# tsurumeso/vocal-remover

Hardware: AMD Instinct MI355X
Metric: spectrogram-frames/sec (inference, CascadedNet n_fft=2048) (higher is better)
Workload: dtype f32; 1 GPU; configs[1]: 30 s stereo 44.1 kHz synthetic song, STFT -> 11 crops of 256 frames in one device batch -> predict_mask -> stitch -> mask apply -> iSTFT x2; n_fft=2048, hop=1024, cropsize=256, parallelism=replicas x1 (songs shard, no collective), input_residency=inputs resident in HBM when the timed region starts

## Files before the change

vocal-remover_amd/csrc/kernels.h:

```cpp
#pragma once
#include "vr_common.h"

namespace vr {

struct HeadDst {
    float* p;
    long long dN, dC, dH;
    int w_lo, w_hi;
    int pad_rows;
    float* const* items;
    const int* item_pitch;
};
void launch_head_sigmoid(const Tensor& x, const float* w , const HeadDst& d, hipStream_t st);
void launch_head_complex(const Tensor& x, const float* w , const HeadDst& d, hipStream_t st);
int launch_squeeze_conv(const Tensor& x, const float* w , float* out, float* part, bool dry, hipStream_t st,
                        const float* epi = nullptr);

void launch_avgpool_h(const Tensor& x, float* out, hipStream_t st);

struct BNFoldDesc { const float *w, *b, *rm, *rv; float* affine; int C; int bcast; };
void launch_bn_fold_eval(const BNFoldDesc* d_descs, int ndesc, int maxC, float eps, hipStream_t st);
struct BNFinalizeArgs {
    const float* part; int nparts; int pstride;
    double count;
// ... 119 lines not shown
void launch_head_loss(const Tensor& x, const float* w, const float* X, const float* Y, int bins, float gscale,
                      float* dlogit, float* mask_out, float* loss_part, float* loss_out, float loss_scale, hipStream_t st);
void launch_head_bwd(const float* dmask, const float* mask, int N, int H, int W, int bins, float* dlogit, hipStream_t st);
void launch_head_loss_complex(const Tensor& x, const float* w, const float* X, const float* Y, int bins, float gscale,
                              float* dlogit, float* mask_out, float* loss_part, float* loss_out, float loss_scale, hipStream_t st);
void launch_head_bwd_complex(const Tensor& x, const float* w, const float* dmask, int bins, float* dlogit, hipStream_t st);
struct MagL1 {};
void launch_head_mag_l1(const Tensor& x, const float* w, const float* X, const float* Y, int bins, float* mask_out, float* loss_part,
                        float* loss_out, float loss_scale, hipStream_t st);
struct FlipDesc { const float* w; float* wt; int Cin, Cout, KK, CinPad, CoutPad; };
void launch_flip_transpose(const FlipDesc* d_descs, int n, hipStream_t st);
void launch_adam(float* p, const float* g, float* m, float* v, long long n, double lr, double b1, double b2, double eps,
                 long long step, double gscale, hipStream_t st);
void launch_channel_sum(const float* d, int N, int C, int W, float* out, int accumulate, hipStream_t st);
void launch_f32_to_bf16(const float* x, unsigned short* y, long long n, hipStream_t st);
void launch_bf16_to_f32(const unsigned short* x, float* y, long long n, hipStream_t st);

void launch_mul_crop(const float* x, float* m, bool cplx, long long rows, int T, int Wm, int off, hipStream_t st);
int l1_crop_blocks();
enum L1CropForm { L1_CROP_REAL = 0, L1_CROP_COMPLEX = 1, L1_CROP_MAG = 2 };
void launch_l1_crop(L1CropForm form, const float* pred, const float* y, long long rows, int T, int Wm, int off, float* part, float* loss,
                    hipStream_t st);

struct FFTPlan { int n_fft; int log2n; float2* twiddle; float* window; };
void launch_stft(const FFTPlan& pl, const float* wave, long long L, int hop, int T, float2* spec, hipStream_t st);
void launch_istft(const FFTPlan& pl, const float2* spec, int hop, int T, float* frames, float* wave, hipStream_t st);
bool istft_masked_available(const FFTPlan& pl, int hop);
void launch_istft_masked(const FFTPlan& pl, const float2* spec, int hop, int T, const float* mask_a, int Wa, const float* mask_b,
                         int Wb, int shift, const float* wgt, int which, float* wave, hipStream_t st);
struct PcmIn { const uint8_t* bytes; int channels; int fmt; };
void launch_stft_pcm(const FFTPlan& pl, const PcmIn& in, long long L, int T, float2* spec, hipStream_t st);
void launch_istft_masked_pcm16(const FFTPlan& pl, const float2* spec, int hop, int T, bool cplx, const float* mask_a, int Wa,
                               const float* mask_b, int Wb, int shift, const float* wgt, int which, int16_t* out, hipStream_t st);
void launch_mag_pad(const float2* spec, int bins, int T, float* mag_pad, int Wpad, int pad_l,
                    unsigned* stats, hipStream_t st);
void launch_coef_affine(unsigned* stats, int rows, int mode, float* aff, hipStream_t st);
void launch_coef_complex(unsigned* stats, int rows, int mode, float2* inv, hipStream_t st);
void launch_pack_complex(const float2* spec, int N, int bins, int T, float* dst, int Wdst, int pad_l, const float2* scale,
                         hipStream_t st);
void launch_apply_mask(const float2* spec, int bins, int T, const float* mask_a, int Wa,
                       const float* mask_b, int Wb, int shift, const float* wgt, float2* y, float2* v, hipStream_t st);
void launch_frame_min(int bins, int T, const float* mask_a, int Wa, const float* mask_b, int Wb, int shift, float* fmin,
                      hipStream_t st);
void launch_apply_mask_complex(const float2* spec, int bins, int T, const float2* mask_a, int Wa, const float2* mask_b, int Wb,
                               int shift, const float* wgt, float2* y, float2* v, hipStream_t st);
void launch_istft_masked_complex(const FFTPlan& pl, const float2* spec, int hop, int T, const float2* mask_a, int Wa,
                                 const float2* mask_b, int Wb, int shift, const float* wgt, int which, float* wave, hipStream_t st);
// ... 155 lines not shown
```

vocal-remover_amd/csrc/model.h:

```cpp
#pragma once
#include <chrono>
#include <deque>
#include <functional>
#include <map>
#include <memory>
#include <string>
#include <vector>

#include "kernels.h"
#include "weight_forms.h"

namespace vr {

struct Arena {
    char* base = nullptr;
    size_t cap = 0, off = 0, peak = 0;
    bool dry = false;
    void* alloc(size_t bytes) {
        const size_t a = (off + 255) & ~size_t(255);
        off = a + bytes;
        if (off > peak) peak = off;
        if (dry) return reinterpret_cast<void*>(uintptr_t(256));
        if (off > cap) throw Error(-4, "workspace arena overflow (planning bug)");
        return base + a;
// ... 250 lines not shown
    int net_w_lo = 0, net_w_hi = 0;
    void set_option(const std::string& name, int value);
    void reset_adam_state();
    void profile_end(double* conv_ms, double* conv_flops, double* conv_bytes, int* launches);

    hipStream_t stream = nullptr;
    hipStream_t side_stream = nullptr;
    hipEvent_t ev_fork = nullptr, ev_join = nullptr;
    bool band_fork_active = false;
    bool gs_clear_pending = false;
    bool wgrad_on_side = false;
    struct Lane { hipStream_t main = nullptr, side = nullptr; hipEvent_t fork = nullptr, join = nullptr, start = nullptr, done = nullptr; Arena ws; };
    std::vector<Lane> lanes;
    void swap_lane(int i);

private:
    float* p_arena = nullptr; size_t p_floats = 0;
    float* b_arena = nullptr; size_t b_floats = 0;
    Arena ws;
    Arena io;
    void ensure_ws(size_t bytes);
    int plan_B = -1, plan_T = -1; bool plan_training = false; size_t plan_peak = 0;
    void ensure_io(size_t bytes);

    std::deque<BN> bns;
    std::vector<BN*> bn_list;
    struct PendingConv { ConvArgs a; ConvShape shp; double flops, bytes; bool stats; BNFinalizeArgs fin; BN* bn; };
    std::vector<PendingConv>* conv_sink = nullptr;
    int x3d_mode = 2;
    int conv_w_lo = 0, conv_w_hi = 0;
    int x3s_mode = x3s_default();
    static int x3s_default() { const char* e = getenv("VR_CONV_X3S"); return (e && atoi(e) == 0) ? 0 : 1; }
    FormStore form_store;
    void hold_form(FormId f, const std::vector<Conv*>& convs, Wino6Want w6, FormStore& s);
    void fill_form(FormId f, const std::vector<Conv*>& convs, Wino6Want w6, FormStore& s, bool single);
    FormSelect form_select() const { return FormSelect{mfma_mode, training, train_wino, x3d_mode, x3s_mode, dry}; }
    std::vector<WgReduceDesc> wred_host, wred_sent;
    WgReduceDesc* wred_dev = nullptr;
    size_t wred_cap = 0;
    void flush_wgrad_sums();
    static long long x3_batch_max_elems(const std::vector<X3WDesc>& descs);
    static int x3_batch_max_cout_pad(const std::vector<X3WDesc>& descs);
    static long long wino_batch_max_elems(const std::vector<WinoWDesc>& descs, bool split6);
    static long long s2w_batch_max_elems(const std::vector<S2WDesc>& descs);
    void refresh_forms(bool with_dgrad);
    BNFoldDesc* d_fold = nullptr;
// ... 131 lines not shown
```

vocal-remover_amd/csrc/model.hip:

```cpp
#include "pcm.h"
#include "model.h"

#include <algorithm>
#include <chrono>
#include <cmath>
#include <cstdlib>
#include <cstring>

namespace vr {

static inline int round_up(int v, int m) { return (v + m - 1) / m * m; }

Param* Model::add_param(const std::string& key, std::vector<int64_t> shape, ParamKind kind, bool trainable) {
    params.emplace_back();
    Param* p = &params.back();
    p->key = key;
    p->shape = std::move(shape);
    p->kind = kind;
    p->trainable = trainable;
    p->numel = 1;
    for (auto d : p->shape) p->numel *= (size_t)d;
    p->dev_numel = p->numel;
    if (kind == PK_CONV) {
        p->Cout = (int)p->shape[0];
// ... 123 lines not shown
    build_basenet(nets_[2], "stg2_low_band_net.0", nout / 4 + nin, nout, nin_lstm / 2, nout_lstm);
    build_cba(tail2, "stg2_low_band_net.1", nout, nout / 2, 1, 1, 0, 0, 1, 1, 0.f);
    build_basenet(nets_[3], "stg2_high_band_net", nout / 4 + nin, nout / 2, nin_lstm / 2, nout_lstm / 2);
    build_basenet(nets_[4], "stg3_full_band_net", 3 * nout / 4 + nin, nout, nin_lstm, nout_lstm);
    out_w = add_param("out.weight", {nin, nout, 1, 1}, PK_PLAIN, true);
    aux_out_w = add_param("aux_out.weight", {nin, 3 * nout / 4, 1, 1}, PK_PLAIN, true);
    finalize_layout();

    plan.n_fft = n_fft;
    plan.log2n = 0;
    while ((1 << plan.log2n) < n_fft) ++plan.log2n;
    std::vector<float2> tw(n_fft / 2);
    std::vector<float> win(n_fft);
    const double PI = 3.14159265358979323846;
    for (int k = 0; k < n_fft / 2; ++k) {
        const double a = -2.0 * PI * k / n_fft;
        tw[k] = make_float2((float)std::cos(a), (float)std::sin(a));
    }
    for (int i = 0; i < n_fft; ++i) win[i] = (float)(0.5 - 0.5 * std::cos(2.0 * PI * i / n_fft));
    VR_HIP(hipMalloc(&plan.twiddle, tw.size() * sizeof(float2)));
    VR_HIP(hipMalloc(&plan.window, win.size() * sizeof(float)));
    VR_HIP(hipMemcpy(plan.twiddle, tw.data(), tw.size() * sizeof(float2), hipMemcpyHostToDevice));
    VR_HIP(hipMemcpy(plan.window, win.data(), win.size() * sizeof(float), hipMemcpyHostToDevice));
}

void Model::finalize_layout() {
    size_t poff = 0, boff = 0;
    auto bump = [](size_t& o, size_t n) { size_t a = (o + 63) & ~size_t(63); o = a + n; return a; };
    for (auto& p : params) {
        if (p.kind == PK_NBT || p.alias_of) continue;
        if (p.trainable) p.off = bump(poff, p.dev_numel);
        else p.off = bump(boff, p.dev_numel);
    }
    std::vector<size_t> aff_off(bn_list.size()), sm_off(bn_list.size()), si_off(bn_list.size());
    for (size_t i = 0; i < bn_list.size(); ++i) {
        BN* b = bn_list[i];
        const int rows = b->bcast ? b->bcast : b->C;
        aff_off[i] = bump(boff, (size_t)rows * 2);
        sm_off[i] = bump(boff, (size_t)b->C);
        si_off[i] = bump(boff, (size_t)b->C);
    }
    size_t aspp_off[5];
    for (int i = 0; i < 5; ++i) aspp_off[i] = bump(boff, (size_t)4 * 8 * nets_[i].c * 2);
    p_floats = poff + 64; b_floats = boff + 64;
    VR_HIP(hipMalloc(&p_arena, p_floats * sizeof(float)));
    VR_HIP(hipMalloc(&b_arena, b_floats * sizeof(float)));
// ... 20 lines not shown
    for (BN* b : bn_list) {
        std::vector<float> ones(b->C, 1.f);
        VR_HIP(hipMemcpy(b->w->dev, ones.data(), b->C * sizeof(float), hipMemcpyHostToDevice));
        VR_HIP(hipMemcpy(b->rv->dev, ones.data(), b->C * sizeof(float), hipMemcpyHostToDevice));
    }
    std::vector<BNFoldDesc> descs;
    for (BN* b : bn_list) descs.push_back(BNFoldDesc{b->w->dev, b->b->dev, b->rm->dev, b->rv->dev, b->affine, b->C, b->bcast});
    VR_HIP(hipMalloc(&d_fold, descs.size() * sizeof(BNFoldDesc)));
    VR_HIP(hipMemcpy(d_fold, descs.data(), descs.size() * sizeof(BNFoldDesc), hipMemcpyHostToDevice));
    affine_dirty = true;
}

Model::~Model() {
    if (launch_prof && !prof_owned_by_this_thread(launch_prof)) prof_abandon(launch_prof);
    else { if (g_launch_prof == launch_prof) g_launch_prof = nullptr; prof_destroy(launch_prof); }
    int prev_dev = -1;
    if (hipGetDevice(&prev_dev) != hipSuccess) prev_dev = -1;
    hipSetDevice(device);
    struct Back { int d; ~Back() { if (d >= 0) hipSetDevice(d); } } back{prev_dev};
    try { comm_destroy(); } catch (...) {}
    hipFree(wire_buf);
    if (stream) hipStreamSynchronize(stream);
    hipFree(p_arena); hipFree(b_arena); hipFree(d_fold);
    hipFree(ws.base); hipFree(io.base); hipFree(gs.base); form_store.release(); hipFree(aug_buf); hipFree(wred_dev);
    for (BaseNetL& B : nets_) hipFree(B.lstm.bias_sum);
    hipFree(g_arena); hipFree(m_arena); hipFree(v_arena); hipFree(dropout_buf);
    hipFree(plan.twiddle); hipFree(plan.window);
    for (Lane& l : lanes) {
        hipStreamSynchronize(l.main); hipStreamSynchronize(l.side);
        hipStreamDestroy(l.main); hipStreamDestroy(l.side);
        hipEventDestroy(l.fork); hipEventDestroy(l.join); hipEventDestroy(l.start); hipEventDestroy(l.done);
        hipFree(l.ws.base);
    }
    if (side_stream) { hipStreamSynchronize(side_stream); hipStreamDestroy(side_stream); hipEventDestroy(ev_fork); hipEventDestroy(ev_join); }
    if (stream) hipStreamDestroy(stream);
}

void Model::set_param(const std::string& key, const void* host, const int64_t* shape, int ndim) {
    auto it = by_key.find(key);
    VR_CHECK(it != by_key.end(), -2, "unknown parameter key: " + key);
    Param& p = *it->second;
    VR_CHECK((size_t)ndim == p.shape.size(), -2, "shape rank mismatch for " + key);
    for (int i = 0; i < ndim; ++i) VR_CHECK(shape[i] == p.shape[i], -2, "shape mismatch for " + key);
    DeviceGuard dev_guard(device);
    VR_HIP(hipStreamSynchronize(stream));
    if (p.kind == PK_NBT) { p.nbt = *static_cast<const int64_t*>(host); return; }
// ... 81 lines not shown

void Model::set_option(const std::string& name, int value) {
    plan_peak = 0;
    if (name == "train_winograd") train_wino = value != 0;
    else if (name == "serial_exec") serial = value != 0;
    else if (name == "params_dirty") affine_dirty = true;
    else if (name == "mfma_bf16") { mfma_mode = value != 0 ? 1 : default_mfma_mode; affine_dirty = true; }
    else if (name == "mfma_mode") {
        if (value < -1 || value > 3) throw Error(-2, "mfma_mode: 0, 1, 2, 3 or -1 (default)");
        mfma_mode = value < 0 ? default_mfma_mode : value; affine_dirty = true;
    }
    else if (name == "conv_x3d") {
        if (value < -1 || value > 2) throw Error(-2, "conv_x3d: 0, 1, 2 or -1 (default)");
        x3d_mode = value < 0 ? 2 : value;
    }
    else if (name == "conv_x3s") {
        if (value < -1 || value > 1) throw Error(-2, "conv_x3s: 0, 1 or -1 (default)");
        x3s_mode = value < 0 ? x3s_default() : value;
    }
    else if (name == "crop_window") crop_window = value != 0;
    else if (name == "fuse_tail") fuse_tail = value != 0;
    else if (name == "lstm_gemm") lstm_gemm = value != 0;
    else if (name == "aspp_pool_fused") aspp_pool_fused = value != 0;
    else if (name == "complex_train") {
        if (!is_complex) throw Error(-2, "complex_train: this handle predicts a magnitude mask; the option belongs to complex-mask handles (VR_CREATE_COMPLEX)");
        complex_train = value != 0;
        if (!complex_train && loss_kind != 0) set_loss(0, 0.01);
        graph_valid = false;
    }
    else if (name == "adam_reset") reset_adam_state();
    else if (name == "hip_graph" || name == "conv_x3p" || name == "wgrad_x3h" || name == "conv_x3b") {
        static std::string told;
        if (told.find("|" + name + "|") == std::string::npos) {
            told += "|" + name + "|";
            fprintf(stderr, "libvr_mi355: option '%s' was retired with its kernel (tools/experiments/README.md); ignored\n", name.c_str());
        }
    }
    else throw Error(-2, "unknown option: " + name);
}

void Model::hold_form(FormId f, const std::vector<Conv*>& convs, Wino6Want w6, FormStore& s) {
    if (s.arena[f]) return;
    auto room = [&](const Conv* L) {
        const FormSpec sp = form_spec(f, *L, mfma_mode, w6);
        return sp.held ? (sp.bytes + 255) & ~size_t(255) : size_t(0);
    };
// ... 89 lines not shown
    ws.base = nullptr; ws.cap = 0;
    const size_t want = bytes + (bytes >> 4) + (1 << 20);
    VR_HIP(hipMalloc(reinterpret_cast<void**>(&ws.base), want));
    ws.cap = want;
}

void Model::swap_lane(int i) {
    Lane& l = lanes[i];
    std::swap(stream, l.main);
    std::swap(side_stream, l.side);
    std::swap(ev_fork, l.fork);
    std::swap(ev_join, l.join);
    std::swap(ws, l.ws);
}

void Model::ensure_io(size_t bytes) {
    if (bytes <= io.cap) return;
    VR_HIP(hipStreamSynchronize(stream));
    if (io.base) VR_HIP(hipFree(io.base));
    io.base = nullptr; io.cap = 0;
    const size_t want = bytes + (bytes >> 4) + (1 << 20);
    VR_HIP(hipMalloc(reinterpret_cast<void**>(&io.base), want));
    io.cap = want;
}

double Model::conv_alg_bytes(const Conv& L, const ConvArgs& a, int N, bool batch_as_h) const {
    return 4.0 * ((double)a.N * L.Cin * a.Hin * a.Win + (double)N * L.Cout * (batch_as_h ? 1 : a.Hout) * a.Wout +
                  (double)L.Cin * L.KS * L.KS * L.Cout);
}

void Model::record_begin(int kind, double flops) {
    if (!profiling || dry) return;
    (void)kind;
    prof_note(flops, 0.0, true, "conv");
}
void Model::record_note(double bytes, const char* tag) {
    if (!profiling || dry || !g_launch_prof) return;
    prof_note_update(bytes, tag);
}
void Model::record_end() {
    if (!profiling || dry) return;
    prof_note_clear();
}

void Model::profile_begin() {
    VR_CHECK(!launch_prof || prof_owned_by_this_thread(launch_prof), -3, "vr_profile_begin: a profile opened by another thread is still open");
// ... 1132 lines not shown
    const int most = solo ? std::max(sg[0].patches[0], sg[0].patches[1]) : crops_n;
    const int bs = (batchsize <= 0) ? most : std::min(batchsize, most);
    const bool tiled = many_tiled_available(plan, hop);

    DeviceGuard dev_guard(device);
    std::vector<SongSeg> tab((size_t)n_songs);
    std::vector<float*> stage_in((size_t)n_songs), stage_y((size_t)n_songs), stage_v((size_t)n_songs);
    SongSeg* tab_d = nullptr; int2* crops_d = nullptr;
    std::vector<PcmIn> pin(pcm ? (size_t)n_songs : 0);
    PcmIn* pin_d = nullptr;
    std::vector<WaveEval> evt(eval ? (size_t)n_songs : 0);
    std::vector<float*> stage_inst(eval ? (size_t)n_songs : 0);
    WaveEval* evt_d = nullptr;
    std::vector<PseudoSeg> pst(pseudo ? (size_t)n_songs : 0);
    std::vector<float*> stage_pinst(pseudo ? (size_t)n_songs : 0);
    PseudoSeg* pst_d = nullptr;
    double pcm_bytes = 0.0;
    auto in_bytes = [&](int s) {
        return pcm ? (size_t)L[s] * pcm_channels[s] * pcm_sample_bytes(pcm_fmt[s]) : (waves ? (size_t)2 * L[s] : sg[s].spec_f) * sizeof(float);
    };
    unsigned long long* part = nullptr;
    float *aff = nullptr, *mask = nullptr, *gather = nullptr, *fmin_d = nullptr, *wgt_d = nullptr, *frames = nullptr;
    const size_t crop_f = (size_t)nin * max_bin * cropsize;
    auto carve = [&](Arena& A) {
        tab_d = static_cast<SongSeg*>(A.alloc(sizeof(SongSeg) * n_songs));
        crops_d = static_cast<int2*>(A.alloc(sizeof(int2) * crops_n));
        if (pcm) pin_d = static_cast<PcmIn*>(A.alloc(sizeof(PcmIn) * n_songs));
        if (eval) evt_d = static_cast<WaveEval*>(A.alloc(sizeof(WaveEval) * n_songs));
        if (pseudo) pst_d = static_cast<PseudoSeg*>(A.alloc(sizeof(PseudoSeg) * n_songs));
        part = static_cast<unsigned long long*>(A.alloc((size_t)n_songs * 2 * bins * 16));
        aff = A.allocf((size_t)n_songs * 4);
        mask = A.allocf((size_t)E * 2 * bins * W);
        gather = A.allocf((size_t)bs * crop_f + 4096);
        if (post) { fmin_d = A.allocf((size_t)sum_T); wgt_d = A.allocf((size_t)sum_T); }
        if (waves && !tiled) frames = A.allocf((size_t)2 * max_T * n_fft);
        for (int s = 0; s < n_songs; ++s) {
            const Song& g = sg[s];
            SongSeg& t = tab[s];
            t = SongSeg{};
            t.T = g.T;
            t.mcol_a = g.crop0[0] * roi;
            t.mcol_b = tta ? g.crop0[1] * roi + roi / 2 : 0;
            stage_in[s] = in_on_dev ? nullptr : A.allocf(in_bytes(s) / 4 + (pcm ? 1 : 0));
            const float* src = in_on_dev ? in[s] : stage_in[s];
            if (pseudo) {
                stage_pinst[s] = in_on_dev ? nullptr : A.allocf(in_bytes(s) / 4);
                const float* isrc = in_on_dev ? pseudo->inst[s] : stage_pinst[s];
                PseudoSeg& q = pst[s];
                q = PseudoSeg{};
// ... 37 lines not shown
                t.spec = reinterpret_cast<float2*>(const_cast<float*>(src));
                stage_y[s] = out_on_dev ? y[s] : A.allocf(g.spec_f);
                stage_v[s] = out_on_dev ? v[s] : A.allocf(g.spec_f);
                t.y = reinterpret_cast<float2*>(stage_y[s]); t.v = reinterpret_cast<float2*>(stage_v[s]);
            }
        }
    };
    Arena dry;
    dry.dry = true;
    carve(dry);
    ensure_io(dry.peak + 65536);
    io.reset();
    carve(io);
    std::vector<int2> crops((size_t)crops_n);
    int frame0 = 0;
    for (int s = 0; s < n_songs; ++s) {
        tab[s].frame0 = frame0;
        if (post) tab[s].fmin = fmin_d + frame0;
        frame0 += sg[s].T;
        for (int ps = 0; ps < (tta ? 2 : 1); ++ps)
            for (int i = 0; i < sg[s].patches[ps]; ++i)
                crops[(size_t)sg[s].crop0[ps] + i] = make_int2(s, i * roi - sg[s].pad_l - (ps ? roi / 2 : 0));
    }
    VR_HIP(hipMemcpyAsync(tab_d, tab.data(), sizeof(SongSeg) * n_songs, hipMemcpyHostToDevice, stream));
    VR_HIP(hipMemcpyAsync(crops_d, crops.data(), sizeof(int2) * crops_n, hipMemcpyHostToDevice, stream));
    if (pcm) {
        VR_HIP(hipMemcpyAsync(pin_d, pin.data(), sizeof(PcmIn) * n_songs, hipMemcpyHostToDevice, stream));
        for (int s = 0; s < n_songs; ++s) pcm_bytes += (double)in_bytes(s);
    }
    if (!in_on_dev)
        for (int s = 0; s < n_songs; ++s)
            VR_HIP(hipMemcpyAsync(stage_in[s], in[s], in_bytes(s), hipMemcpyHostToDevice, stream));
    if (eval) {
        VR_HIP(hipMemcpyAsync(evt_d, evt.data(), sizeof(WaveEval) * n_songs, hipMemcpyHostToDevice, stream));
        if (!in_on_dev)
            for (int s = 0; s < n_songs; ++s)
                VR_HIP(hipMemcpyAsync(stage_inst[s], eval->inst[s], in_bytes(s), hipMemcpyHostToDevice, stream));
    }
    if (pseudo) {
        VR_HIP(hipMemcpyAsync(pst_d, pst.data(), sizeof(PseudoSeg) * n_songs, hipMemcpyHostToDevice, stream));
        if (!in_on_dev)
            for (int s = 0; s < n_songs; ++s)
                VR_HIP(hipMemcpyAsync(stage_pinst[s], pseudo->inst[s], in_bytes(s), hipMemcpyHostToDevice, stream));
    }
    if (pseudo) {
        if (waves) launch_stft_pseudo_many(plan, tab_d, pst_d, n_songs, max_T, (double)sum_L, (double)sum_T, stream);
        else launch_pseudo_diff_many(tab_d, pst_d, n_songs, bins, (double)sum_T, stream);
    } else if (waves) {
// ... 559 lines not shown
```

vocal-remover_amd/csrc/stft.hip:

```cpp
#include "kernels.h"
#include "pcm.h"

#include <cfloat>
#include <cstdlib>
#include <cstring>
#include <type_traits>

namespace vr {

template <class SRC> constexpr bool kSongTable = std::is_same<SRC, const SongSeg>::value;
template <class SRC> constexpr bool kStream = std::is_same<SRC, const StreamSeg>::value;
template <class SRC> using StreamLocal = typename std::conditional<kStream<SRC>, StreamSeg, int>::type;
template <class SRC> constexpr bool kPair = std::is_same<SRC, const WavePair>::value;
template <class SRC> using PairLocal = typename std::conditional<kPair<SRC>, WavePair, int>::type;
template <class SRC> constexpr bool kTriple = std::is_same<SRC, const WaveTriple>::value;
template <class SRC> using TripleLocal = typename std::conditional<kTriple<SRC>, WaveTriple, int>::type;

__device__ __forceinline__ float stream_sample(const StreamSeg& sg, int ch, long long p) {
    if (p < 0 || p >= sg.L) return 0.f;
    return p < sg.blk_base ? sg.tail[(long long)ch * sg.tail_pitch + (p - sg.tail_base)] : sg.blk[(long long)ch * sg.blk_pitch + (p - sg.blk_base)];
}

__device__ __forceinline__ float2 cmul(float2 a, float2 b) {
    return make_float2(a.x * b.x - a.y * b.y, a.x * b.y + a.y * b.x);
}

__device__ __forceinline__ float2 sub_rounded(float2 a, float2 b) {
#pragma clang fp contract(off)
// ... 32 lines not shown
    for (int i = threadIdx.x; i < n; i += blockDim.x) {
        const long long p = start + i;
        const float v = (p >= 0 && p < L) ? wv[p] * pl.window[i] : 0.f;
        const int r = __brev((unsigned)i) >> (32 - pl.log2n);
        xs[r] = make_float2(v, 0.f);
    }
    fft_lds(xs, pl.twiddle, n, pl.log2n);
    const int bins = n / 2 + 1;
    for (int k = threadIdx.x; k < bins; k += blockDim.x)
        spec[((long long)ch * bins + k) * T + t] = xs[k];
}

void launch_stft(const FFTPlan& pl, const float* wave, long long L, int hop, int T, float2* spec, hipStream_t st);
static int tile_frames(const FFTPlan& pl, int extra_floats);
static bool tiled_signal_path(const FFTPlan& pl, int hop);
void launch_stft_tiled(const FFTPlan& pl, const float* wave, long long L, int T, float2* spec, hipStream_t st);

void launch_stft(const FFTPlan& pl, const float* wave, long long L, int hop, int T, float2* spec, hipStream_t st) {
    if (tiled_signal_path(pl, hop)) { launch_stft_tiled(pl, wave, L, T, spec, st); return; }
    VR_LAUNCH(stft_kernel, dim3(T, 2), dim3(256), pl.n_fft * sizeof(float2), st, pl, wave, L, hop, T, spec);
    VR_HIP(hipGetLastError());
}

__device__ __forceinline__ void fft_lds_sub(float2* x, const float2* __restrict__ tw, int n, int log2n, int twshift, int tid,
                                            int nt) {
    const int half_n = n >> 1;
    for (int s = 0; s < log2n; ++s) {
        const int half = 1 << s;
        __syncthreads();
        for (int b = tid; b < half_n; b += nt) {
            const int pos = b & (half - 1);
            const int i = ((b >> s) << (s + 1)) + pos;
            const int j = i + half;
            const float2 w = tw[(pos << (log2n - 1 - s)) << twshift];
            const float2 t = cmul(w, x[j]);
            const float2 u = x[i];
            x[i] = make_float2(u.x + t.x, u.y + t.y);
            x[j] = make_float2(u.x - t.x, u.y - t.y);
        }
    }
    __syncthreads();
}

constexpr int TG = 4;

template <class A> __device__ __forceinline__ A pcm_first(A a) { return a; }
template <class D, class... T> struct FirstOr { using type = D; };
template <class D, class A, class... T> struct FirstOr<D, A, T...> { using type = A; };

struct WaveF32In {
    const float* wv;
    __device__ __forceinline__ float at(long long p) const { return wv[p]; }
};
struct WavePcmIn {
    PcmIn in;
    int ch;
    __device__ __forceinline__ float at(long long p) const { return pcm_decode(in.bytes, in.fmt, in.channels, p, ch); }
};
struct WaveGradIn {
    const float* yw;
    const float* pw;
    const float* win;
// ... 20 lines not shown
        const float ws = fmaf(w0, w0, w2 * w2);
        const float a = fmaf(cy, yw[p], fmaf(cp, pw[p], cx * xw[p]));
        return ws > FLT_MIN ? a / ws : a;
    }
};
struct WaveF32Out {
    static constexpr bool kInterleaved = false;
    static __device__ __forceinline__ void put(float* w, long long pitch, int ch, long long p, int i, float v) { w[(long long)ch * pitch + p + i] = v; }
};
struct WavePcm16Out {
    static constexpr bool kInterleaved = true;
    static __device__ __forceinline__ void put(float* w, long long, int ch, long long p, int i, float v) {
        reinterpret_cast<int16_t*>(w)[(p + i) * 2 + ch] = pcm16_from_float(v);
    }
};

template <class SRC = const float, class... PCM>
__global__ __launch_bounds__(1024) void stft_tile_kernel(FFTPlan pl, SRC* __restrict__ wave, long long L, int T, int F,
                                                         float2* __restrict__ spec, PCM... pcm) {
    constexpr bool kGrad3 = std::is_same<typename FirstOr<void, PCM...>::type, WaveGrad3>::value;
    constexpr bool kGrad = std::is_same<typename FirstOr<void, PCM...>::type, WaveGrad>::value || kGrad3;
    constexpr bool kPseudo = std::is_same<typename FirstOr<void, PCM...>::type, const PseudoSeg*>::value;
    constexpr bool kPcm = sizeof...(PCM) == 1 && !kGrad && !kPseudo;
    static_assert(!kPseudo || kSongTable<SRC>, "the pair form is a song-table form");
    static_assert(sizeof...(PCM) <= 1 && !(sizeof...(PCM) == 1 && kStream<SRC>), "one PCM source at most, none for streams");
    extern __shared__ __attribute__((aligned(16))) float2 lds2[];
    const int n = pl.n_fft, M = n >> 1, bins = M + 1, hop = M, logM = pl.log2n - 1;
    const int g = threadIdx.x >> 8, tid = threadIdx.x & 255;
    float2* zs = lds2 + (size_t)g * M;
    float2* tile = lds2 + (size_t)TG * M;
    int t0 = blockIdx.x * F;
    const int ch = blockIdx.y;
    typename std::conditional<kPcm, WavePcmIn, typename std::conditional<kGrad3, WaveGrad3In,
                              typename std::conditional<kGrad, WaveGradIn, WaveF32In>::type>::type>::type in;
    typename std::conditional<kGrad3, WaveGrad3, typename std::conditional<kGrad, WaveGrad, int>::type>::type gd{};
    StreamLocal<SRC> ss{};
    typename std::conditional<kPseudo, PseudoSeg, int>::type ps{};
    const float* mix_wv = nullptr;
    if constexpr (kStream<SRC>) {
        ss = wave[blockIdx.z];
        if (blockIdx.x > 0 && t0 >= ss.T - ss.t_new) return;
        t0 += ss.t_new; T = ss.T;
        in.wv = nullptr;
    } else if constexpr (kSongTable<SRC>) {
        const SongSeg sg = wave[blockIdx.z];
        if (t0 >= sg.T) return;
// ... 11 lines not shown
                                             (double)gd.sums[4], (double)gd.sums[5]);
        in.xw = gd.x_wave + (long long)ch * L; in.yw = gd.y_wave + (long long)ch * L; in.pw = gd.p_wave + (long long)ch * L;
        in.win = pl.window; in.M = M;
        in.cy = (float)((double)gd.sdr_scale * c.cy); in.cp = (float)((double)gd.sdr_scale * c.cp); in.cx = (float)((double)gd.sdr_scale * c.cx);
    } else if constexpr (kGrad) {
        gd = pcm_first(pcm...);
        const double a = (double)gd.sums[0], p = sqrt((double)gd.sums[1]), q = sqrt((double)gd.sums[2]), D = p * q + 1e-8;
        in.yw = gd.y_wave + (long long)ch * L; in.pw = gd.p_wave + (long long)ch * L; in.win = pl.window; in.M = M;
        in.alpha = (float)(-(double)gd.sdr_scale / D);
        in.beta = q > 0.0 ? (float)((double)gd.sdr_scale * a * p / (q * D * D)) : 0.f;
    } else {
        if constexpr (kPcm) in.in = pcm_first(pcm...);
        else in.wv = wave + (long long)ch * L;
    }
    if constexpr (kPcm) in.ch = ch < in.in.channels ? ch : in.in.channels - 1;
    const int nf = (T - t0) < F ? (T - t0) : F;
    int pass = 0;
second_pass:
    for (int f0 = 0; f0 < nf; f0 += TG) {
        const int f = f0 + g;
        const bool live = f < nf;
        if (live) {
            const long long start = (long long)(t0 + f) * hop - M;
            for (int m = tid; m < M; m += 256) {
                const long long p = start + 2 * m;
                float v0, v1;
                if constexpr (kStream<SRC>) {
                    v0 = stream_sample(ss, ch, p) * pl.window[2 * m];
                    v1 = stream_sample(ss, ch, p + 1) * pl.window[2 * m + 1];
                } else {
                    v0 = (p >= 0 && p < L) ? in.at(p) * pl.window[2 * m] : 0.f;
                    v1 = (p + 1 >= 0 && p + 1 < L) ? in.at(p + 1) * pl.window[2 * m + 1] : 0.f;
                }
                zs[__brev((unsigned)m) >> (32 - logM)] = make_float2(v0, v1);
            }
        }
        fft_lds_sub(zs, pl.twiddle, M, logM, 1, tid, 256);
        if (live) {
            for (int k = tid; k < bins; k += 256) {
                const float2 zk = zs[k & (M - 1)], zm = zs[(M - k) & (M - 1)];
                const float2 e = make_float2(0.5f * (zk.x + zm.x), 0.5f * (zk.y - zm.y));
                const float2 b = make_float2(0.5f * (zk.x - zm.x), 0.5f * (zk.y + zm.y));
                const float2 w = k < M ? pl.twiddle[k] : make_float2(-1.f, 0.f);
                const float2 wb = cmul(w, b);
                if constexpr (kPseudo) {
                    const float2 xv = make_float2(e.x + wb.y, e.y - wb.x);
                    tile[k * F + f] = pass == 1 ? sub_rounded(xv, tile[k * F + f]) : xv;
                } else {
                    tile[k * F + f] = make_float2(e.x + wb.y, e.y - wb.x);
                }
            }
        }
// ... 358 lines not shown
        }
        __syncthreads();
        if (threadIdx.x < 6) {
            float s = 0.f;
            for (int w = 0; w < 16; ++w) s += red[w * 6 + threadIdx.x];
            tr.part[((long long)blockIdx.y * gridDim.x + blockIdx.x) * 6 + threadIdx.x] = s;
        }
    }
    if constexpr (kStream<SRC>) {
        if (t0 + nf == ss.t_done) {
            float* cout = ss.carry_out + (long long)(which * 2 + ch) * M;
            for (int i = threadIdx.x; i < M; i += 1024) cout[i] = prev[i];
        }
    }
}

static int tile_frames(const FFTPlan& pl, int extra_floats) {
    const int M = pl.n_fft / 2, bins = M + 1;
    long long budget = 150 * 1024 - (long long)TG * M * 8 - (long long)extra_floats * 4;
    int F = (int)(budget / ((long long)bins * 8));
    return F > 17 ? 17 : F;
}

static bool tiled_signal_path(const FFTPlan& pl, int hop) {
    static const bool on = !getenv("VR_NO_TILED_STFT");
    return on && hop * 2 == pl.n_fft && pl.n_fft >= 128 && tile_frames(pl, pl.n_fft / 2) >= 3;
}

template <bool CPLX, class... OUT>
static void launch_istft_tile(const FFTPlan& pl, const float2* spec, int hop, int T, const float* mask_a, int Wa, const float* mask_b,
                              int Wb, int shift, const float* wgt, int which, float* wave, hipStream_t st) {
    const int M = pl.n_fft / 2, bins = M + 1;
    const long long out_len = (long long)hop * (T - 1);
    if (out_len <= 0) return;
    const int F = tile_frames(pl, M);
    const int S = F - 1;
    const size_t lds = (size_t)TG * M * 8 + (size_t)bins * F * 8 + (size_t)M * 4;
    static std::atomic<unsigned long long> attr_done{0};
    ensure_lds_attr(attr_done, reinterpret_cast<const void*>(istft_tile_kernel<CPLX, const float2, OUT...>), 160 * 1024);
    prof_note(0.0, 2.0 * ((double)bins * T * (8.0 + (CPLX ? 8.0 : 4.0) * (mask_b ? 2 : 1)) + (sizeof...(OUT) ? 2.0 : 4.0) * (double)out_len));
    VR_LAUNCH((istft_tile_kernel<CPLX, const float2, OUT...>), dim3((unsigned)((T - 1 + S - 1) / S), 2), dim3(1024), lds, st, pl, spec, T, S, mask_a, Wa,
              mask_b, Wb, shift, wgt, which, wave, out_len);
    VR_HIP(hipGetLastError());
}

void launch_istft_masked(const FFTPlan& pl, const float2* spec, int hop, int T, const float* mask_a, int Wa, const float* mask_b,
                         int Wb, int shift, const float* wgt, int which, float* wave, hipStream_t st) {
    launch_istft_tile<false>(pl, spec, hop, T, mask_a, Wa, mask_b, Wb, shift, wgt, which, wave, st);
}

void launch_istft_masked_pcm16(const FFTPlan& pl, const float2* spec, int hop, int T, bool cplx, const float* mask_a, int Wa,
                               const float* mask_b, int Wb, int shift, const float* wgt, int which, int16_t* out, hipStream_t st) {
    float* w = reinterpret_cast<float*>(out);
    if (cplx) launch_istft_tile<true, WavePcm16Out>(pl, spec, hop, T, mask_a, Wa, mask_b, Wb, shift, wgt, which, w, st);
    else launch_istft_tile<false, WavePcm16Out>(pl, spec, hop, T, mask_a, Wa, mask_b, Wb, shift, wgt, which, w, st);
}

void launch_istft_masked_complex(const FFTPlan& pl, const float2* spec, int hop, int T, const float2* mask_a, int Wa,
                                 const float2* mask_b, int Wb, int shift, const float* wgt, int which, float* wave, hipStream_t st) {
    launch_istft_tile<true>(pl, spec, hop, T, reinterpret_cast<const float*>(mask_a), Wa, reinterpret_cast<const float*>(mask_b), Wb,
// ... 121 lines not shown
    const long long p = (long long)blockIdx.x * blockDim.x + threadIdx.x;
    const int ch = blockIdx.y;
    if (p >= out_len) return;
    const int n = pl.n_fft;
    const long long q = p + n / 2;
    long long t_hi = q / hop;
    if (t_hi > T - 1) t_hi = T - 1;
    long long t_lo = (q - n + hop) / hop;
    if (q - n + 1 <= 0) t_lo = 0;
    if (t_lo < 0) t_lo = 0;
    float acc = 0.f, wss = 0.f;
    for (long long t = t_lo; t <= t_hi; ++t) {
        const int i = (int)(q - t * hop);
        if (i < 0 || i >= n) continue;
        acc += frames[((long long)ch * T + t) * n + i];
        const float w = pl.window[i];
        wss = fmaf(w, w, wss);
    }
    wave[(long long)ch * out_len + p] = (wss > FLT_MIN) ? acc / wss : acc;
}

void launch_stft_tiled(const FFTPlan& pl, const float* wave, long long L, int T, float2* spec, hipStream_t st) {
    const int M = pl.n_fft / 2, bins = M + 1;
    int F = tile_frames(pl, 0);
    if (F > 16) F = 16;
    F = F / TG * TG;
    const size_t lds = (size_t)TG * M * 8 + (size_t)bins * F * 8;
    static std::atomic<unsigned long long> attr_done{0};
    ensure_lds_attr(attr_done, reinterpret_cast<const void*>(stft_tile_kernel<>), 160 * 1024);
    prof_note(0.0, 2.0 * (4.0 * (double)L + 8.0 * (double)bins * T));
    VR_LAUNCH((stft_tile_kernel<>), dim3((unsigned)((T + F - 1) / F), 2), dim3(1024), lds, st, pl, wave, L, T, F, spec);
    VR_HIP(hipGetLastError());
}

void launch_stft_pcm(const FFTPlan& pl, const PcmIn& in, long long L, int T, float2* spec, hipStream_t st) {
    const int M = pl.n_fft / 2, bins = M + 1;
    int F = tile_frames(pl, 0);
    if (F > 16) F = 16;
    F = F / TG * TG;
    const size_t lds = (size_t)TG * M * 8 + (size_t)bins * F * 8;
    static std::atomic<unsigned long long> attr_done{0};
    ensure_lds_attr(attr_done, reinterpret_cast<const void*>(stft_tile_kernel<const float, PcmIn>), 160 * 1024);
    prof_note(0.0, (double)pcm_sample_bytes(in.fmt) * in.channels * (double)L + 2.0 * 8.0 * (double)bins * T);
    VR_LAUNCH((stft_tile_kernel<const float, PcmIn>), dim3((unsigned)((T + F - 1) / F), 2), dim3(1024), lds, st, pl, (const float*)nullptr, L, T, F,
              spec, in);
    VR_HIP(hipGetLastError());
}

bool istft_masked_available(const FFTPlan& pl, int hop) { return tiled_signal_path(pl, hop); }

void launch_istft(const FFTPlan& pl, const float2* spec, int hop, int T, float* frames, float* wave, hipStream_t st) {
    if (tiled_signal_path(pl, hop)) {
        launch_istft_masked(pl, spec, hop, T, nullptr, 0, nullptr, 0, 0, nullptr, 0, wave, st);
        return;
    }
    VR_LAUNCH(istft_frame_kernel, dim3(T, 2), dim3(256), pl.n_fft * sizeof(float2), st, pl, spec, T, frames);
    VR_HIP(hipGetLastError());
    const long long out_len = (long long)hop * (T - 1);
    if (out_len > 0) {
        VR_LAUNCH(istft_ola_kernel, dim3((unsigned)((out_len + 255) / 256), 2), dim3(256), 0, st, pl, frames,
                           hop, T, out_len, wave);
        VR_HIP(hipGetLastError());
    }
// ... 353 lines not shown
    VR_HIP(hipGetLastError());
}

void launch_frame_min_complex(int bins, int T, const float2* mask_a, int Wa, const float2* mask_b, int Wb, int shift, float* fmin,
                              hipStream_t st) {
    VR_LAUNCH((frame_min_kernel<true>), dim3((T + 63) / 64), dim3(256), 0, st, 2 * bins, T, reinterpret_cast<const float*>(mask_a), Wa,
              reinterpret_cast<const float*>(mask_b), Wb, shift, fmin);
    VR_HIP(hipGetLastError());
}

void launch_apply_mask_complex(const float2* spec, int bins, int T, const float2* mask_a, int Wa, const float2* mask_b, int Wb,
                               int shift, const float* wgt, float2* y, float2* v, hipStream_t st) {
    const long long total = 2LL * bins * T;
    VR_LAUNCH((apply_mask_kernel<true>), dim3((unsigned)((total + 255) / 256)), dim3(256), 0, st, spec, bins, T,
              reinterpret_cast<const float*>(mask_a), Wa, reinterpret_cast<const float*>(mask_b), Wb, shift, wgt, y, v);
    VR_HIP(hipGetLastError());
}

bool many_tiled_available(const FFTPlan& pl, int hop) { return tiled_signal_path(pl, hop); }

void launch_stft_many(const FFTPlan& pl, const SongSeg* songs, int n_songs, int max_T, double sum_L, double sum_T, hipStream_t st,
                      const PcmIn* pcm, double pcm_bytes) {
    const int M = pl.n_fft / 2, bins = M + 1;
    int F = tile_frames(pl, 0);
    if (F > 16) F = 16;
    F = F / TG * TG;
    const size_t lds = (size_t)TG * M * 8 + (size_t)bins * F * 8;
    if (pcm) {
        static std::atomic<unsigned long long> attr_pcm{0};
        ensure_lds_attr(attr_pcm, reinterpret_cast<const void*>(stft_tile_kernel<const SongSeg, const PcmIn*>), 160 * 1024);
        prof_note(0.0, pcm_bytes + 2.0 * 8.0 * (double)bins * sum_T);
        VR_LAUNCH((stft_tile_kernel<const SongSeg, const PcmIn*>), dim3((unsigned)((max_T + F - 1) / F), 2, n_songs), dim3(1024), lds, st, pl, songs, 0LL,
                  0, F, (float2*)nullptr, pcm);
        VR_HIP(hipGetLastError());
        return;
    }
    static std::atomic<unsigned long long> attr_done{0};
    ensure_lds_attr(attr_done, reinterpret_cast<const void*>(stft_tile_kernel<const SongSeg>), 160 * 1024);
    prof_note(0.0, 2.0 * (4.0 * sum_L + 8.0 * (double)bins * sum_T));
    VR_LAUNCH((stft_tile_kernel<const SongSeg>), dim3((unsigned)((max_T + F - 1) / F), 2, n_songs), dim3(1024), lds, st, pl, songs, 0LL, 0, F, nullptr);
    VR_HIP(hipGetLastError());
}

void launch_song_stats(const SongSeg* songs, int n_songs, int bins, double sum_T, unsigned long long* part, hipStream_t st) {
    prof_note(0.0, 2.0 * (double)bins * 8.0 * sum_T);
    VR_LAUNCH((mag_pad_kernel<false, const SongSeg>), dim3(2 * bins, n_songs), dim3(256), 0, st, songs, 0, nullptr, 0, 0, part, bins, nullptr);
    VR_HIP(hipGetLastError());
}

void launch_song_coef(const unsigned long long* part, int n_songs, int rows, int mode, bool cplx, float* aff, hipStream_t st) {
// ... 16 lines not shown
void launch_frame_min_many(const SongSeg* songs, int n_songs, int max_T, int bins, const float* mask, int W, int tta, bool cplx,
                           hipStream_t st) {
    const dim3 grid((max_T + 63) / 64, n_songs);
    const float* mb = tta ? mask : nullptr;
    if (cplx) VR_LAUNCH((frame_min_kernel<true, const SongSeg>), grid, dim3(256), 0, st, 2 * bins, 0, mask, W, mb, W, 0, songs);
    else VR_LAUNCH((frame_min_kernel<false, const SongSeg>), grid, dim3(256), 0, st, 2 * bins, 0, mask, W, mb, W, 0, songs);
    VR_HIP(hipGetLastError());
}

void launch_apply_mask_many(const SongSeg* songs, int n_songs, int max_T, int bins, const float* mask, int W, int tta, bool cplx,
                            const float* wgt, hipStream_t st) {
    const long long total = 2LL * bins * max_T;
    const dim3 grid((unsigned)((total + 255) / 256), n_songs);
    const float* mb = tta ? mask : nullptr;
    if (cplx) VR_LAUNCH((apply_mask_kernel<true, const SongSeg>), grid, dim3(256), 0, st, songs, bins, 0, mask, W, mb, W, 0, wgt, nullptr, nullptr);
    else VR_LAUNCH((apply_mask_kernel<false, const SongSeg>), grid, dim3(256), 0, st, songs, bins, 0, mask, W, mb, W, 0, wgt, nullptr, nullptr);
    VR_HIP(hipGetLastError());
}

void launch_istft_masked_many(const FFTPlan& pl, const SongSeg* songs, int n_songs, int max_T, double sum_T, const float* mask, int W, int tta,
                              bool cplx, const float* wgt, int which, hipStream_t st, bool pcm16) {
    const int M = pl.n_fft / 2, bins = M + 1;
    if (max_T < 2) return;
    const int F = tile_frames(pl, M);
    const int S = F - 1;
    const size_t lds = (size_t)TG * M * 8 + (size_t)bins * F * 8 + (size_t)M * 4;
    const dim3 grid((unsigned)((max_T - 1 + S - 1) / S), 2, n_songs);
    prof_note(0.0, 2.0 * ((double)bins * sum_T * (8.0 + (cplx ? 8.0 : 4.0) * (tta ? 2 : 1)) + (pcm16 ? 2.0 : 4.0) * (double)M * sum_T));
    const float* mb = tta ? mask : nullptr;
    if (pcm16) {
        if (cplx) {
            static std::atomic<unsigned long long> attr_done{0};
            ensure_lds_attr(attr_done, reinterpret_cast<const void*>(istft_tile_kernel<true, const SongSeg, WavePcm16Out>), 160 * 1024);
            VR_LAUNCH((istft_tile_kernel<true, const SongSeg, WavePcm16Out>), grid, dim3(1024), lds, st, pl, songs, 0, S, mask, W, mb, W, 0, wgt, which, nullptr, 0LL);
        } else {
            static std::atomic<unsigned long long> attr_done{0};
            ensure_lds_attr(attr_done, reinterpret_cast<const void*>(istft_tile_kernel<false, const SongSeg, WavePcm16Out>), 160 * 1024);
            VR_LAUNCH((istft_tile_kernel<false, const SongSeg, WavePcm16Out>), grid, dim3(1024), lds, st, pl, songs, 0, S, mask, W, mb, W, 0, wgt, which, nullptr, 0LL);
        }
        VR_HIP(hipGetLastError());
        return;
    }
    if (cplx) {
        static std::atomic<unsigned long long> attr_done{0};
        ensure_lds_attr(attr_done, reinterpret_cast<const void*>(istft_tile_kernel<true, const SongSeg>), 160 * 1024);
        VR_LAUNCH((istft_tile_kernel<true, const SongSeg>), grid, dim3(1024), lds, st, pl, songs, 0, S, mask, W, mb, W, 0, wgt, which, nullptr, 0LL);
    } else {
        static std::atomic<unsigned long long> attr_done{0};
        ensure_lds_attr(attr_done, reinterpret_cast<const void*>(istft_tile_kernel<false, const SongSeg>), 160 * 1024);
// ... 150 lines not shown
```

Before: 192,200 spectrogram-frames/sec.

## Pick STFT/iSTFT frame tiles by CU occupancy and tune FFT stages

The STFT and iSTFT frame tile size is now chosen from the number of workgroups relative to the CU count, and it can also be forced through an env var or option. The FFT's early butterfly stages now run per wavefront with wave barriers instead of full-block barriers. The f32 STFT loads sample pairs with float2. The song and crop tables go to the device in one copy from a single pinned host buffer instead of two pageable copies. The aim is better GPU fill for short songs and fewer barriers and transfers, at the cost of more code paths and a risk of LDS hazards in the wave-local FFT stages.

```diff
diff --git a/vocal-remover_amd/csrc/kernels.h b/vocal-remover_amd/csrc/kernels.h
--- a/vocal-remover_amd/csrc/kernels.h
+++ b/vocal-remover_amd/csrc/kernels.h
@@ -165,7 +165,8 @@
 void launch_l1_crop(L1CropForm form, const float* pred, const float* y, long long rows, int T, int Wm, int off, float* part, float* loss,
                     hipStream_t st);
 
-struct FFTPlan { int n_fft; int log2n; float2* twiddle; float* window; };
+struct FFTPlan { int n_fft; int log2n; float2* twiddle; float* window; int tile_fwd; int tile_inv; };
+bool tile_frames_valid(const FFTPlan& pl, bool inverse, int F);
 void launch_stft(const FFTPlan& pl, const float* wave, long long L, int hop, int T, float2* spec, hipStream_t st);
 void launch_istft(const FFTPlan& pl, const float2* spec, int hop, int T, float* frames, float* wave, hipStream_t st);
 bool istft_masked_available(const FFTPlan& pl, int hop);
diff --git a/vocal-remover_amd/csrc/model.h b/vocal-remover_amd/csrc/model.h
--- a/vocal-remover_amd/csrc/model.h
+++ b/vocal-remover_amd/csrc/model.h
@@ -296,6 +296,8 @@
     void ensure_ws(size_t bytes);
     int plan_B = -1, plan_T = -1; bool plan_training = false; size_t plan_peak = 0;
     void ensure_io(size_t bytes);
+    char* tab_pin = nullptr; size_t tab_pin_cap = 0;
+    char* ensure_tab_pin(size_t bytes);
 
     std::deque<BN> bns;
     std::vector<BN*> bn_list;
diff --git a/vocal-remover_amd/csrc/model.hip b/vocal-remover_amd/csrc/model.hip
--- a/vocal-remover_amd/csrc/model.hip
+++ b/vocal-remover_amd/csrc/model.hip
@@ -169,6 +169,12 @@
     VR_HIP(hipMalloc(&plan.window, win.size() * sizeof(float)));
     VR_HIP(hipMemcpy(plan.twiddle, tw.data(), tw.size() * sizeof(float2), hipMemcpyHostToDevice));
     VR_HIP(hipMemcpy(plan.window, win.data(), win.size() * sizeof(float), hipMemcpyHostToDevice));
+    static const int env_fwd = getenv("VR_STFT_TILE_FRAMES") ? atoi(getenv("VR_STFT_TILE_FRAMES")) : 0;
+    static const int env_inv = getenv("VR_ISTFT_TILE_FRAMES") ? atoi(getenv("VR_ISTFT_TILE_FRAMES")) : 0;
+    VR_CHECK(tile_frames_valid(plan, false, env_fwd) && tile_frames_valid(plan, true, env_inv), -2,
+             "VR_STFT_TILE_FRAMES / VR_ISTFT_TILE_FRAMES: 0 or a frame tile that fits the LDS (forward: a multiple of 4)");
+    plan.tile_fwd = env_fwd;
+    plan.tile_inv = env_inv;
 }
 
 void Model::finalize_layout() {
@@ -235,6 +241,7 @@
     hipFree(wire_buf);
     if (stream) hipStreamSynchronize(stream);
     hipFree(p_arena); hipFree(b_arena); hipFree(d_fold);
+    if (tab_pin) (void)hipHostFree(tab_pin);
     hipFree(ws.base); hipFree(io.base); hipFree(gs.base); form_store.release(); hipFree(aug_buf); hipFree(wred_dev);
     for (BaseNetL& B : nets_) hipFree(B.lstm.bias_sum);
     hipFree(g_arena); hipFree(m_arena); hipFree(v_arena); hipFree(dropout_buf);
@@ -362,6 +369,11 @@
     else if (name == "fuse_tail") fuse_tail = value != 0;
     else if (name == "lstm_gemm") lstm_gemm = value != 0;
     else if (name == "aspp_pool_fused") aspp_pool_fused = value != 0;
+    else if (name == "stft_tile_frames" || name == "istft_tile_frames") {
+        const bool inverse = name[0] == 'i';
+        if (!tile_frames_valid(plan, inverse, value)) throw Error(-2, name + ": 0 (the rule) or a frame tile that fits the LDS" + (inverse ? "" : ", a multiple of 4"));
+        (inverse ? plan.tile_inv : plan.tile_fwd) = value;
+    }
     else if (name == "complex_train") {
         if (!is_complex) throw Error(-2, "complex_train: this handle predicts a magnitude mask; the option belongs to complex-mask handles (VR_CREATE_COMPLEX)");
         complex_train = value != 0;
@@ -497,6 +509,16 @@
     const size_t want = bytes + (bytes >> 4) + (1 << 20);
     VR_HIP(hipMalloc(reinterpret_cast<void**>(&io.base), want));
     io.cap = want;
+}
+
+char* Model::ensure_tab_pin(size_t bytes) {
+    if (bytes <= tab_pin_cap) return tab_pin;
+    if (tab_pin) VR_HIP(hipHostFree(tab_pin));
+    tab_pin = nullptr; tab_pin_cap = 0;
+    const size_t want = bytes + (bytes >> 1) + 4096;
+    VR_HIP(hipHostMalloc(reinterpret_cast<void**>(&tab_pin), want, hipHostMallocDefault));
+    tab_pin_cap = want;
+    return tab_pin;
 }
 
 double Model::conv_alg_bytes(const Conv& L, const ConvArgs& a, int N, bool batch_as_h) const {
@@ -1675,9 +1697,10 @@
     unsigned long long* part = nullptr;
     float *aff = nullptr, *mask = nullptr, *gather = nullptr, *fmin_d = nullptr, *wgt_d = nullptr, *frames = nullptr;
     const size_t crop_f = (size_t)nin * max_bin * cropsize;
+    const size_t crops_at = (sizeof(SongSeg) * n_songs + 15) & ~size_t(15);
     auto carve = [&](Arena& A) {
-        tab_d = static_cast<SongSeg*>(A.alloc(sizeof(SongSeg) * n_songs));
-        crops_d = static_cast<int2*>(A.alloc(sizeof(int2) * crops_n));
+        tab_d = static_cast<SongSeg*>(A.alloc(crops_at + sizeof(int2) * crops_n));
+        crops_d = reinterpret_cast<int2*>(reinterpret_cast<char*>(tab_d) + crops_at);
         if (pcm) pin_d = static_cast<PcmIn*>(A.alloc(sizeof(PcmIn) * n_songs));
         if (eval) evt_d = static_cast<WaveEval*>(A.alloc(sizeof(WaveEval) * n_songs));
         if (pseudo) pst_d = static_cast<PseudoSeg*>(A.alloc(sizeof(PseudoSeg) * n_songs));
@@ -1761,8 +1784,13 @@
             for (int i = 0; i < sg[s].patches[ps]; ++i)
                 crops[(size_t)sg[s].crop0[ps] + i] = make_int2(s, i * roi - sg[s].pad_l - (ps ? roi / 2 : 0));
     }
-    VR_HIP(hipMemcpyAsync(tab_d, tab.data(), sizeof(SongSeg) * n_songs, hipMemcpyHostToDevice, stream));
-    VR_HIP(hipMemcpyAsync(crops_d, crops.data(), sizeof(int2) * crops_n, hipMemcpyHostToDevice, stream));
+    {
+        const size_t bytes = crops_at + sizeof(int2) * crops_n;
+        char* pinned = ensure_tab_pin(bytes);
+        memcpy(pinned, tab.data(), sizeof(SongSeg) * n_songs);
+        memcpy(pinned + crops_at, crops.data(), sizeof(int2) * crops_n);
+        VR_HIP(hipMemcpyAsync(tab_d, pinned, bytes, hipMemcpyHostToDevice, stream));
+    }
     if (pcm) {
         VR_HIP(hipMemcpyAsync(pin_d, pin.data(), sizeof(PcmIn) * n_songs, hipMemcpyHostToDevice, stream));
         for (int s = 0; s < n_songs; ++s) pcm_bytes += (double)in_bytes(s);
diff --git a/vocal-remover_amd/csrc/stft.hip b/vocal-remover_amd/csrc/stft.hip
--- a/vocal-remover_amd/csrc/stft.hip
+++ b/vocal-remover_amd/csrc/stft.hip
@@ -4,6 +4,7 @@
 #include <cfloat>
 #include <cstdlib>
 #include <cstring>
+#include <initializer_list>
 #include <type_traits>
 
 namespace vr {
@@ -82,22 +83,36 @@
     VR_HIP(hipGetLastError());
 }
 
+__device__ __forceinline__ void fft_butterfly(float2* x, const float2* __restrict__ tw, int log2n, int twshift, int s, int b) {
+    const int half = 1 << s;
+    const int pos = b & (half - 1);
+    const int i = ((b >> s) << (s + 1)) + pos;
+    const int j = i + half;
+    const float2 w = tw[(pos << (log2n - 1 - s)) << twshift];
+    const float2 t = cmul(w, x[j]);
+    const float2 u = x[i];
+    x[i] = make_float2(u.x + t.x, u.y + t.y);
+    x[j] = make_float2(u.x - t.x, u.y - t.y);
+}
+
 __device__ __forceinline__ void fft_lds_sub(float2* x, const float2* __restrict__ tw, int n, int log2n, int twshift, int tid,
                                             int nt) {
     const int half_n = n >> 1;
-    for (int s = 0; s < log2n; ++s) {
-        const int half = 1 << s;
+    int s = 0;
+    if (nt == 256 && n >= 256) {
+        const int per_wave = n >> 3, b0 = (tid >> 6) * per_wave, lane = tid & 63;
         __syncthreads();
-        for (int b = tid; b < half_n; b += nt) {
-            const int pos = b & (half - 1);
-            const int i = ((b >> s) << (s + 1)) + pos;
-            const int j = i + half;
-            const float2 w = tw[(pos << (log2n - 1 - s)) << twshift];
-            const float2 t = cmul(w, x[j]);
-            const float2 u = x[i];
-            x[i] = make_float2(u.x + t.x, u.y + t.y);
-            x[j] = make_float2(u.x - t.x, u.y - t.y);
-        }
+        for (; s < log2n - 2; ++s) {
+            if (s > 0) {
+                asm volatile("s_waitcnt lgkmcnt(0)" ::: "memory");
+                __builtin_amdgcn_wave_barrier();
+            }
+            for (int b = lane; b < per_wave; b += 64) fft_butterfly(x, tw, log2n, twshift, s, b0 + b);
+        }
+    }
+    for (; s < log2n; ++s) {
+        __syncthreads();
+        for (int b = tid; b < half_n; b += nt) fft_butterfly(x, tw, log2n, twshift, s, b);
     }
     __syncthreads();
 }
@@ -164,6 +179,7 @@
     constexpr bool kGrad = std::is_same<typename FirstOr<void, PCM...>::type, WaveGrad>::value || kGrad3;
     constexpr bool kPseudo = std::is_same<typename FirstOr<void, PCM...>::type, const PseudoSeg*>::value;
     constexpr bool kPcm = sizeof...(PCM) == 1 && !kGrad && !kPseudo;
+    constexpr bool kF32 = !kPcm && !kGrad && !kStream<SRC>;
     static_assert(!kPseudo || kSongTable<SRC>, "the pair form is a song-table form");
     static_assert(sizeof...(PCM) <= 1 && !(sizeof...(PCM) == 1 && kStream<SRC>), "one PCM source at most, none for streams");
     extern __shared__ __attribute__((aligned(16))) float2 lds2[];
@@ -221,12 +237,21 @@
         const bool live = f < nf;
         if (live) {
             const long long start = (long long)(t0 + f) * hop - M;
+            bool pair_ok = false;
+            if constexpr (kF32) pair_ok = (reinterpret_cast<uintptr_t>(in.wv) & 7) == 0;
             for (int m = tid; m < M; m += 256) {
                 const long long p = start + 2 * m;
                 float v0, v1;
                 if constexpr (kStream<SRC>) {
                     v0 = stream_sample(ss, ch, p) * pl.window[2 * m];
                     v1 = stream_sample(ss, ch, p + 1) * pl.window[2 * m + 1];
+                } else if (kF32 && pair_ok && p >= 0 && p + 1 < L) {
+                    if constexpr (kF32) {
+                        const float2 s = *reinterpret_cast<const float2*>(in.wv + p);
+                        const float2 w = *reinterpret_cast<const float2*>(pl.window + 2 * m);
+                        v0 = s.x * w.x;
+                        v1 = s.y * w.y;
+                    }
                 } else {
                     v0 = (p >= 0 && p < L) ? in.at(p) * pl.window[2 * m] : 0.f;
                     v1 = (p + 1 >= 0 && p + 1 < L) ? in.at(p + 1) * pl.window[2 * m + 1] : 0.f;
@@ -631,6 +656,45 @@
     return F > 17 ? 17 : F;
 }
 
+static size_t tile_lds_bytes(const FFTPlan& pl, bool inverse, int F) {
+    const int M = pl.n_fft / 2, bins = M + 1;
+    return (size_t)TG * M * 8 + (size_t)bins * F * 8 + (inverse ? (size_t)M * 4 : 0);
+}
+
+static int tile_frames_max(const FFTPlan& pl, bool inverse) {
+    if (inverse) return tile_frames(pl, pl.n_fft / 2);
+    const int F = tile_frames(pl, 0);
+    return (F > 16 ? 16 : F) / TG * TG;
+}
+
+bool tile_frames_valid(const FFTPlan& pl, bool inverse, int F) {
+    if (F == 0) return true;
+    if (F < TG || F > tile_frames_max(pl, inverse)) return false;
+    return inverse || F % TG == 0;
+}
+
+static int tile_plan(const FFTPlan& pl, bool inverse, int max_T, int pairs) {
+    const int forced = inverse ? pl.tile_inv : pl.tile_fwd;
+    const int top = tile_frames_max(pl, inverse);
+    if (forced) return forced;
+    static const int cus = [] {
+        int dev = 0, n = 0;
+        if (hipGetDevice(&dev) != hipSuccess || hipDeviceGetAttribute(&n, hipDeviceAttributeMultiprocessorCount, dev) != hipSuccess || n < 1) n = 256;
+        return n;
+    }();
+    const int units = inverse ? max_T - 1 : max_T;
+    int best = top;
+    long long best_cost = -1;
+    for (int F : {top, 2 * TG, TG}) {
+        if (F > top || (F == top && best_cost >= 0)) continue;
+        const int step = inverse ? F - 1 : F;
+        const long long wgs = (long long)((units + step - 1) / step) * pairs;
+        const long long cost = (long long)((F + TG - 1) / TG) * ((wgs + cus - 1) / cus);
+        if (best_cost < 0 || cost < best_cost) { best = F; best_cost = cost; }
+    }
+    return best;
+}
+
 static bool tiled_signal_path(const FFTPlan& pl, int hop) {
     static const bool on = !getenv("VR_NO_TILED_STFT");
     return on && hop * 2 == pl.n_fft && pl.n_fft >= 128 && tile_frames(pl, pl.n_fft / 2) >= 3;
@@ -642,9 +706,9 @@
     const int M = pl.n_fft / 2, bins = M + 1;
     const long long out_len = (long long)hop * (T - 1);
     if (out_len <= 0) return;
-    const int F = tile_frames(pl, M);
+    const int F = tile_plan(pl, true, T, 2);
     const int S = F - 1;
-    const size_t lds = (size_t)TG * M * 8 + (size_t)bins * F * 8 + (size_t)M * 4;
+    const size_t lds = tile_lds_bytes(pl, true, F);
     static std::atomic<unsigned long long> attr_done{0};
     ensure_lds_attr(attr_done, reinterpret_cast<const void*>(istft_tile_kernel<CPLX, const float2, OUT...>), 160 * 1024);
     prof_note(0.0, 2.0 * ((double)bins * T * (8.0 + (CPLX ? 8.0 : 4.0) * (mask_b ? 2 : 1)) + (sizeof...(OUT) ? 2.0 : 4.0) * (double)out_len));
@@ -812,10 +876,8 @@
 
 void launch_stft_tiled(const FFTPlan& pl, const float* wave, long long L, int T, float2* spec, hipStream_t st) {
     const int M = pl.n_fft / 2, bins = M + 1;
-    int F = tile_frames(pl, 0);
-    if (F > 16) F = 16;
-    F = F / TG * TG;
-    const size_t lds = (size_t)TG * M * 8 + (size_t)bins * F * 8;
+    const int F = tile_plan(pl, false, T, 2);
+    const size_t lds = tile_lds_bytes(pl, false, F);
     static std::atomic<unsigned long long> attr_done{0};
     ensure_lds_attr(attr_done, reinterpret_cast<const void*>(stft_tile_kernel<>), 160 * 1024);
     prof_note(0.0, 2.0 * (4.0 * (double)L + 8.0 * (double)bins * T));
@@ -825,10 +887,8 @@
 
 void launch_stft_pcm(const FFTPlan& pl, const PcmIn& in, long long L, int T, float2* spec, hipStream_t st) {
     const int M = pl.n_fft / 2, bins = M + 1;
-    int F = tile_frames(pl, 0);
-    if (F > 16) F = 16;
-    F = F / TG * TG;
-    const size_t lds = (size_t)TG * M * 8 + (size_t)bins * F * 8;
+    const int F = tile_plan(pl, false, T, 2);
+    const size_t lds = tile_lds_bytes(pl, false, F);
     static std::atomic<unsigned long long> attr_done{0};
     ensure_lds_attr(attr_done, reinterpret_cast<const void*>(stft_tile_kernel<const float, PcmIn>), 160 * 1024);
     prof_note(0.0, (double)pcm_sample_bytes(in.fmt) * in.channels * (double)L + 2.0 * 8.0 * (double)bins * T);
@@ -1228,10 +1288,8 @@
 void launch_stft_many(const FFTPlan& pl, const SongSeg* songs, int n_songs, int max_T, double sum_L, double sum_T, hipStream_t st,
                       const PcmIn* pcm, double pcm_bytes) {
     const int M = pl.n_fft / 2, bins = M + 1;
-    int F = tile_frames(pl, 0);
-    if (F > 16) F = 16;
-    F = F / TG * TG;
-    const size_t lds = (size_t)TG * M * 8 + (size_t)bins * F * 8;
+    const int F = tile_plan(pl, false, max_T, 2 * n_songs);
+    const size_t lds = tile_lds_bytes(pl, false, F);
     if (pcm) {
         static std::atomic<unsigned long long> attr_pcm{0};
         ensure_lds_attr(attr_pcm, reinterpret_cast<const void*>(stft_tile_kernel<const SongSeg, const PcmIn*>), 160 * 1024);
@@ -1294,9 +1352,9 @@
                               bool cplx, const float* wgt, int which, hipStream_t st, bool pcm16) {
     const int M = pl.n_fft / 2, bins = M + 1;
     if (max_T < 2) return;
-    const int F = tile_frames(pl, M);
+    const int F = tile_plan(pl, true, max_T, 2 * n_songs);
     const int S = F - 1;
-    const size_t lds = (size_t)TG * M * 8 + (size_t)bins * F * 8 + (size_t)M * 4;
+    const size_t lds = tile_lds_bytes(pl, true, F);
     const dim3 grid((unsigned)((max_T - 1 + S - 1) / S), 2, n_songs);
     prof_note(0.0, 2.0 * ((double)bins * sum_T * (8.0 + (cplx ? 8.0 : 4.0) * (tta ? 2 : 1)) + (pcm16 ? 2.0 : 4.0) * (double)M * sum_T));
     const float* mb = tta ? mask : nullptr;
```

New measurement: 191,800 spectrogram-frames/sec (median of 2 runs). No clear change (-0.2%).
